# ahmetumutdurmus/zaremba

Measured on NVIDIA H100. Metric: tokens/sec (and valid perplexity) Large-LSTM 1500h at 1/2/4/8 H100 vs ref CPU, higher is better.
Workload: dtype f16 operands, f32 accumulate/state

## Files before the change

zaremba_b200/csrc/optim_tc.cu:

```cuda
#include "tc_kernels.h"

namespace zrb {

struct PackSpec {
    __half* row_img;
    int64_t ld;
    __half* fwd_img;
    int fU, fG, fKc, fKS;
    __half* bwd_img;
    int bUC, bG, bKc, bS;
    int write_g;
    int pdl;
};

__device__ __forceinline__ void pdl_prologue(const PackSpec& sp) {
    if (sp.pdl && threadIdx.x == 0) asm volatile("griddepcontrol.launch_dependents;" ::: "memory");
}
__device__ __forceinline__ void pdl_epilogue(const PackSpec& sp) {
    if (sp.pdl && blockIdx.x == 0 && threadIdx.x == 0) asm volatile("griddepcontrol.wait;" ::: "memory");
}

template <int VEC> struct VecT;
template <> struct VecT<4> { using type = float4; };
template <> struct VecT<2> { using type = float2; };
template <> struct VecT<1> { using type = float; };

template <int VEC>
__device__ __forceinline__ void load_vec(const float* p, float (&v)[VEC]) {
    typename VecT<VEC>::type t = __ldcs(reinterpret_cast<const typename VecT<VEC>::type*>(p));
    const float* f = reinterpret_cast<const float*>(&t);
#pragma unroll
    for (int i = 0; i < VEC; ++i) v[i] = f[i];
}
template <int VEC>
__device__ __forceinline__ void store_halves(__half* dst, const __half (&h)[VEC]) {
    if constexpr (VEC == 1) {
        dst[0] = h[0];
    } else {
#pragma unroll
        for (int x = 0; x < VEC; x += 2) reinterpret_cast<__half2*>(dst)[x >> 1] = __halves2half2(h[x], h[x + 1]);
    }
}

template <int VEC>
__device__ __forceinline__ void store_vec(float* p, const float (&v)[VEC]) {
    typename VecT<VEC>::type t;
    float* f = reinterpret_cast<float*>(&t);
#pragma unroll
    for (int i = 0; i < VEC; ++i) f[i] = v[i];
    __stcs(reinterpret_cast<typename VecT<VEC>::type*>(p), t);
}

struct SgdRule {
    float lr;
    const float* scalars;
    float coef;
    static constexpr bool kMayWriteG = true;
    __device__ __forceinline__ void init() { coef = scalars[1]; }
    template <int VEC>
    __device__ __forceinline__ void apply(int64_t, float (&pv)[VEC], float (&gv)[VEC]) const {
#pragma unroll
        for (int x = 0; x < VEC; ++x) { gv[x] *= coef; pv[x] = sgd_elem(pv[x], gv[x], lr); }
    }
};

template <bool RMS>
struct DynRule {
    const float* tg;
    const float* r;
    DynArgs a;
    float rbar;
    static constexpr bool kMayWriteG = false;
    __device__ __forceinline__ void init() { rbar = RMS ? *a.rbar : 0.f; }
    template <int VEC>
    __device__ __forceinline__ void apply(int64_t off, float (&pv)[VEC], float (&gv)[VEC]) const {
        float tv[VEC], rv[VEC];
        load_vec<VEC>(tg + off, tv);
        if constexpr (RMS) load_vec<VEC>(r + off, rv);
#pragma unroll
        for (int x = 0; x < VEC; ++x)
            pv[x] = dyneval_elem<RMS>(pv[x], gv[x], tv[x], RMS ? rv[x] : 0.f, a.lr, a.lam, a.eps, rbar);
    }
};

template <int VEC, class Rule>
__global__ void update_pack_kernel(float* __restrict__ p, float* __restrict__ g, int rows, int cols, Rule rule,
                                   PackSpec sp) {
    pdl_prologue(sp);
    rule.init();
    const int cv = cols / VEC;
    const int64_t total = (int64_t)rows * cv;
    for (int64_t i = (int64_t)blockIdx.x * blockDim.x + threadIdx.x; i < total; i += (int64_t)gridDim.x * blockDim.x) {
        const int r = (int)(i / cv), c = (int)(i % cv) * VEC;
        const int64_t off = (int64_t)r * cols + c;
        float gv[VEC], pv[VEC];
        load_vec<VEC>(g + off, gv);
        load_vec<VEC>(p + off, pv);
        rule.template apply<VEC>(off, pv, gv);
        if (Rule::kMayWriteG && sp.write_g) store_vec<VEC>(g + off, gv);
        store_vec<VEC>(p + off, pv);
        if (sp.row_img) {
            __half hh[VEC];
#pragma unroll
            for (int x = 0; x < VEC; ++x) hh[x] = __float2half_rn(pv[x]);
            store_halves<VEC>(sp.row_img + (int64_t)r * sp.ld + c, hh);
        }
    }
    pdl_epilogue(sp);
}

template <int VEC, class Rule>
__global__ void update_pack_whh_kernel(float* __restrict__ p, float* __restrict__ g, int H, Rule rule, PackSpec sp) {
    pdl_prologue(sp);
    rule.init();
    const int cv = H / VEC, jb_n = (H + 7) >> 3;
    const int64_t total = (int64_t)4 * jb_n * cv;
    for (int64_t i = (int64_t)blockIdx.x * blockDim.x + threadIdx.x; i < total; i += (int64_t)gridDim.x * blockDim.x) {
        const int c = (int)(i % cv) * VEC;
        const int jb = (int)((i / cv) % jb_n), q = (int)(i / ((int64_t)cv * jb_n));
        const int j0 = jb << 3;
        __half hv[8][VEC];
#pragma unroll
        for (int e = 0; e < 8; ++e) {
            const int j = j0 + e;
            if (j < H) {
                const int64_t off = ((int64_t)q * H + j) * H + c;
                float gv[VEC], pv[VEC];
                load_vec<VEC>(g + off, gv);
                load_vec<VEC>(p + off, pv);
                rule.template apply<VEC>(off, pv, gv);
#pragma unroll
                for (int x = 0; x < VEC; ++x) hv[e][x] = __float2half_rn(pv[x]);
                if (Rule::kMayWriteG && sp.write_g) store_vec<VEC>(g + off, gv);
                store_vec<VEC>(p + off, pv);
                if (sp.row_img) store_halves<VEC>(sp.row_img + ((int64_t)q * H + j) * sp.ld + c, hv[e]);
                if (sp.fwd_img) {
                    const int cluster = j / sp.fU, u = j % sp.fU, row = 4 * u + q;
                    const int kc = c >> 3, cta = cluster * sp.fKS + kc / sp.fKc, kcl = kc % sp.fKc;
                    store_halves<VEC>(sp.fwd_img + (((int64_t)cta * sp.fKc + kcl) * sp.fG + (row >> 3)) * 64 +
                                          (row & 7) * 8 + (c & 7), hv[e]);
                }
            } else {
#pragma unroll
                for (int x = 0; x < VEC; ++x) hv[e][x] = __float2half_rn(0.f);
            }
        }
        if (sp.bwd_img) {
#pragma unroll
            for (int x = 0; x < VEC; ++x) {
                const int cl = (c + x) / sp.bUC, u = (c + x) % sp.bUC;
                uint4 v;
                v.x = (uint32_t)__half_as_ushort(hv[0][x]) | ((uint32_t)__half_as_ushort(hv[1][x]) << 16);
                v.y = (uint32_t)__half_as_ushort(hv[2][x]) | ((uint32_t)__half_as_ushort(hv[3][x]) << 16);
                v.z = (uint32_t)__half_as_ushort(hv[4][x]) | ((uint32_t)__half_as_ushort(hv[5][x]) << 16);
                v.w = (uint32_t)__half_as_ushort(hv[6][x]) | ((uint32_t)__half_as_ushort(hv[7][x]) << 16);
                const int rank = q * sp.bS + jb / sp.bKc, kcl = jb % sp.bKc;
                *reinterpret_cast<uint4*>(sp.bwd_img + ((((int64_t)cl * 4 * sp.bS + rank) * sp.bKc + kcl) * sp.bG) * 64 +
                                          (u >> 3) * 64 + (u & 7) * 8) = v;
            }
        }
    }
    pdl_epilogue(sp);
}

template <int VEC, class Rule>
static int update_pack_launch(float* p, float* g, int rows, int cols, const Rule& rule, const PackSpec& sp, bool whh,
                              cudaStream_t s) {
    int64_t total = whh ? (int64_t)4 * ((cols + 7) / 8) * (cols / VEC) : (int64_t)rows * (cols / VEC);
    const int threads = whh ? 128 : 256;
    int blocks = (int)((total + threads - 1) / threads);
    if (blocks > 132 * 16) blocks = 132 * 16;
    if (sp.pdl) {
        cudaLaunchConfig_t cfg = {};
        cfg.gridDim = dim3(blocks); cfg.blockDim = dim3(threads); cfg.dynamicSmemBytes = 12 * 1024; cfg.stream = s;
        cudaLaunchAttribute at[1];
        at[0].id = cudaLaunchAttributeProgrammaticStreamSerialization;
        at[0].val.programmaticStreamSerializationAllowed = 1;
        cfg.attrs = at; cfg.numAttrs = 1;
        if (whh) ZRB_CUDA(cudaLaunchKernelEx(&cfg, update_pack_whh_kernel<VEC, Rule>, p, g, cols, rule, sp));
        else ZRB_CUDA(cudaLaunchKernelEx(&cfg, update_pack_kernel<VEC, Rule>, p, g, rows, cols, rule, sp));
        count_launch();
        return ZRB_OK;
    }
    if (whh) update_pack_whh_kernel<VEC, Rule><<<blocks, threads, 0, s>>>(p, g, cols, rule, sp);
    else update_pack_kernel<VEC, Rule><<<blocks, threads, 0, s>>>(p, g, rows, cols, rule, sp);
    ZRB_KERNEL_CHECK();
    return ZRB_OK;
}

template <class Rule>
static int update_pack_rule(float* p, float* g, int rows, int cols, const Rule& rule, uintptr_t align, __half* row_img,
                            int64_t ld, __half* fwd_img, const RecPlan* fp, __half* bwd_img, const RecPlan* bp,
                            bool write_g, cudaStream_t s, bool pdl) {
    PackSpec sp;
    sp.write_g = write_g ? 1 : 0;
    sp.pdl = pdl ? 1 : 0;
    sp.row_img = row_img; sp.ld = ld;
    sp.fwd_img = fwd_img; sp.fKS = fp ? fp->KS : 1; sp.fU = fp ? fp->KS * fp->U : 1; sp.fG = fp ? fp->G : 1;
    sp.fKc = fp ? fp->KcS : 1;
    sp.bwd_img = bwd_img; sp.bS = bp ? bp->KS : 1; sp.bUC = bp ? 4 * bp->KS * bp->U : 4; sp.bG = bp ? bp->G : 1;
    sp.bKc = bp ? bp->KcS : 1;
    const bool whh = (fwd_img || bwd_img) && rows == 4 * cols;
    const uintptr_t all = ((uintptr_t)p) | ((uintptr_t)g) | align;
    const bool al16 = (all & 15) == 0, al8 = (all & 7) == 0;
    if (cols % 4 == 0 && al16) return update_pack_launch<4>(p, g, rows, cols, rule, sp, whh, s);
    if (cols % 2 == 0 && al8) return update_pack_launch<2>(p, g, rows, cols, rule, sp, whh, s);
    return update_pack_launch<1>(p, g, rows, cols, rule, sp, whh, s);
}

int update_pack(float* p, float* g, int rows, int cols, float lr, const float* scalars, __half* row_img, int64_t ld,
                __half* fwd_img, const RecPlan* fp, __half* bwd_img, const RecPlan* bp, bool write_g, cudaStream_t s,
                bool pdl) {
    SgdRule rule;
    rule.lr = lr; rule.scalars = scalars; rule.coef = 0.f;
    return update_pack_rule(p, g, rows, cols, rule, 0, row_img, ld, fwd_img, fp, bwd_img, bp, write_g, s, pdl);
}

int update_pack_dyn(float* p, float* g, const float* tg, const float* r, int rows, int cols, const DynArgs& a,
                    __half* row_img, int64_t ld, __half* fwd_img, const RecPlan* fp, __half* bwd_img, const RecPlan* bp,
                    cudaStream_t s) {
    const uintptr_t align = ((uintptr_t)tg) | ((uintptr_t)r);
    if (a.rbar) {
        DynRule<true> rule{tg, r, a, 0.f};
        return update_pack_rule(p, g, rows, cols, rule, align, row_img, ld, fwd_img, fp, bwd_img, bp, false, s, false);
    }
    DynRule<false> rule{tg, nullptr, a, 0.f};
    return update_pack_rule(p, g, rows, cols, rule, align, row_img, ld, fwd_img, fp, bwd_img, bp, false, s, false);
}

}
```

Before: 364,800.

## Tile fused optimizer-update/pack kernels into 8-row blocks with warp-shuffled backward image stores

Replaces the grid-stride loops in the fused SGD/dynamic-eval update-and-pack kernels with a fixed 2D tiling: each thread handles an 8-row by VEC-column tile, batching all loads before the update math. In the W_hh kernel, the four gates q are mapped to adjacent lanes, and the backward-image 16-byte stores are reassembled via byte_perm and a lane-xor-4 shuffle so each thread writes contiguous units. It also adds launch bounds with per-rule min-blocks hints and uses vectorized half2 packing and stores. The aim is more memory-level parallelism and better-coalesced image writes in the per-step optimizer pass, at the cost of register pressure and more complex indexing.

```diff
diff --git a/zaremba_b200/csrc/optim_tc.cu b/zaremba_b200/csrc/optim_tc.cu
--- a/zaremba_b200/csrc/optim_tc.cu
+++ b/zaremba_b200/csrc/optim_tc.cu
@@ -32,14 +32,30 @@
 #pragma unroll
     for (int i = 0; i < VEC; ++i) v[i] = f[i];
 }
-template <int VEC>
-__device__ __forceinline__ void store_halves(__half* dst, const __half (&h)[VEC]) {
+__device__ __forceinline__ void st_v2(__half* dst, uint32_t a, uint32_t b) {
+    asm volatile("st.global.v2.b32 [%0], {%1, %2};" ::"l"(dst), "r"(a), "r"(b));
+}
+__device__ __forceinline__ void st_v4(__half* dst, const uint4& v) {
+    asm volatile("st.global.v4.b32 [%0], {%1, %2, %3, %4};" ::"l"(dst), "r"(v.x), "r"(v.y), "r"(v.z), "r"(v.w));
+}
+
+template <int VEC>
+__device__ __forceinline__ void pack_row(const float (&v)[VEC], uint32_t (&w)[(VEC + 1) / 2]) {
     if constexpr (VEC == 1) {
-        dst[0] = h[0];
+        w[0] = __half_as_ushort(__float2half_rn(v[0]));
     } else {
 #pragma unroll
-        for (int x = 0; x < VEC; x += 2) reinterpret_cast<__half2*>(dst)[x >> 1] = __halves2half2(h[x], h[x + 1]);
-    }
+        for (int k = 0; k < VEC / 2; ++k) {
+            const __half2 h = __floats2half2_rn(v[2 * k], v[2 * k + 1]);
+            w[k] = *reinterpret_cast<const uint32_t*>(&h);
+        }
+    }
+}
+template <int VEC>
+__device__ __forceinline__ void store_halves(__half* dst, const uint32_t (&w)[(VEC + 1) / 2]) {
+    if constexpr (VEC == 4) st_v2(dst, w[0], w[1]);
+    else if constexpr (VEC == 2) *reinterpret_cast<uint32_t*>(dst) = w[0];
+    else *reinterpret_cast<unsigned short*>(dst) = (unsigned short)w[0];
 }
 
 template <int VEC>
@@ -56,6 +72,7 @@
     const float* scalars;
     float coef;
     static constexpr bool kMayWriteG = true;
+    static constexpr int kWhhMinBlocks = 5;
     __device__ __forceinline__ void init() { coef = scalars[1]; }
     template <int VEC>
     __device__ __forceinline__ void apply(int64_t, float (&pv)[VEC], float (&gv)[VEC]) const {
@@ -71,6 +88,7 @@
     DynArgs a;
     float rbar;
     static constexpr bool kMayWriteG = false;
+    static constexpr int kWhhMinBlocks = 4;
     __device__ __forceinline__ void init() { rbar = RMS ? *a.rbar : 0.f; }
     template <int VEC>
     __device__ __forceinline__ void apply(int64_t off, float (&pv)[VEC], float (&gv)[VEC]) const {
@@ -83,80 +101,149 @@
     }
 };
 
+constexpr int kTileRows = 8;
+constexpr int kUpdThreads = 128;
+
 template <int VEC, class Rule>
-__global__ void update_pack_kernel(float* __restrict__ p, float* __restrict__ g, int rows, int cols, Rule rule,
-                                   PackSpec sp) {
+__device__ __forceinline__ void tile_update(const float* __restrict__ p, const float* __restrict__ g, int64_t off,
+                                            int stride, int n, const Rule& rule, float (&pv)[kTileRows][VEC],
+                                            float (&gv)[kTileRows][VEC]) {
+#pragma unroll
+    for (int e = 0; e < kTileRows; ++e) {
+        if (e < n) {
+            load_vec<VEC>(g + off + (int64_t)e * stride, gv[e]);
+            load_vec<VEC>(p + off + (int64_t)e * stride, pv[e]);
+        }
+    }
+#pragma unroll
+    for (int e = 0; e < kTileRows; ++e)
+        if (e < n) rule.template apply<VEC>(off + (int64_t)e * stride, pv[e], gv[e]);
+}
+
+template <int VEC>
+__device__ __forceinline__ void tile_store(float* __restrict__ p, float* __restrict__ g, int64_t off, int stride, int n,
+                                           bool write_g, const float (&pv)[kTileRows][VEC],
+                                           const float (&gv)[kTileRows][VEC]) {
+#pragma unroll
+    for (int e = 0; e < kTileRows; ++e) {
+        if (e < n) {
+            if (write_g) store_vec<VEC>(g + off + (int64_t)e * stride, gv[e]);
+            store_vec<VEC>(p + off + (int64_t)e * stride, pv[e]);
+        }
+    }
+}
+
+
+template <int VEC, class Rule>
+__global__ void __launch_bounds__(kUpdThreads) update_pack_kernel(float* __restrict__ p, float* __restrict__ g, int rows,
+                                                                  int cols, int col_tiles, Rule rule, PackSpec sp) {
     pdl_prologue(sp);
     rule.init();
-    const int cv = cols / VEC;
-    const int64_t total = (int64_t)rows * cv;
-    for (int64_t i = (int64_t)blockIdx.x * blockDim.x + threadIdx.x; i < total; i += (int64_t)gridDim.x * blockDim.x) {
-        const int r = (int)(i / cv), c = (int)(i % cv) * VEC;
-        const int64_t off = (int64_t)r * cols + c;
-        float gv[VEC], pv[VEC];
-        load_vec<VEC>(g + off, gv);
-        load_vec<VEC>(p + off, pv);
-        rule.template apply<VEC>(off, pv, gv);
-        if (Rule::kMayWriteG && sp.write_g) store_vec<VEC>(g + off, gv);
-        store_vec<VEC>(p + off, pv);
+    const unsigned rg = blockIdx.x / (unsigned)col_tiles, ct = blockIdx.x - rg * col_tiles;
+    const int c = (ct * blockDim.x + threadIdx.x) * VEC;
+    const int r0 = rg * kTileRows, n = min(kTileRows, rows - r0);
+    if (c < cols) {
+        const int64_t off = (int64_t)r0 * cols + c;
+        float pv[kTileRows][VEC], gv[kTileRows][VEC];
+        tile_update<VEC>(p, g, off, cols, n, rule, pv, gv);
+        tile_store<VEC>(p, g, off, cols, n, Rule::kMayWriteG && sp.write_g, pv, gv);
         if (sp.row_img) {
-            __half hh[VEC];
-#pragma unroll
-            for (int x = 0; x < VEC; ++x) hh[x] = __float2half_rn(pv[x]);
-            store_halves<VEC>(sp.row_img + (int64_t)r * sp.ld + c, hh);
+#pragma unroll
+            for (int e = 0; e < kTileRows; ++e) {
+                if (e < n) {
+                    uint32_t w[(VEC + 1) / 2];
+                    pack_row<VEC>(pv[e], w);
+                    store_halves<VEC>(sp.row_img + (int64_t)(r0 + e) * sp.ld + c, w);
+                }
+            }
         }
     }
     pdl_epilogue(sp);
 }
 
 template <int VEC, class Rule>
-__global__ void update_pack_whh_kernel(float* __restrict__ p, float* __restrict__ g, int H, Rule rule, PackSpec sp) {
+__global__ void __launch_bounds__(kUpdThreads, Rule::kWhhMinBlocks) update_pack_whh_kernel(float* __restrict__ p, float* __restrict__ g,
+                                                                      int H, int col_tiles, Rule rule, PackSpec sp) {
     pdl_prologue(sp);
     rule.init();
-    const int cv = H / VEC, jb_n = (H + 7) >> 3;
-    const int64_t total = (int64_t)4 * jb_n * cv;
-    for (int64_t i = (int64_t)blockIdx.x * blockDim.x + threadIdx.x; i < total; i += (int64_t)gridDim.x * blockDim.x) {
-        const int c = (int)(i % cv) * VEC;
-        const int jb = (int)((i / cv) % jb_n), q = (int)(i / ((int64_t)cv * jb_n));
-        const int j0 = jb << 3;
-        __half hv[8][VEC];
-#pragma unroll
-        for (int e = 0; e < 8; ++e) {
-            const int j = j0 + e;
-            if (j < H) {
-                const int64_t off = ((int64_t)q * H + j) * H + c;
-                float gv[VEC], pv[VEC];
-                load_vec<VEC>(g + off, gv);
-                load_vec<VEC>(p + off, pv);
-                rule.template apply<VEC>(off, pv, gv);
-#pragma unroll
-                for (int x = 0; x < VEC; ++x) hv[e][x] = __float2half_rn(pv[x]);
-                if (Rule::kMayWriteG && sp.write_g) store_vec<VEC>(g + off, gv);
-                store_vec<VEC>(p + off, pv);
-                if (sp.row_img) store_halves<VEC>(sp.row_img + ((int64_t)q * H + j) * sp.ld + c, hv[e]);
-                if (sp.fwd_img) {
-                    const int cluster = j / sp.fU, u = j % sp.fU, row = 4 * u + q;
-                    const int kc = c >> 3, cta = cluster * sp.fKS + kc / sp.fKc, kcl = kc % sp.fKc;
-                    store_halves<VEC>(sp.fwd_img + (((int64_t)cta * sp.fKc + kcl) * sp.fG + (row >> 3)) * 64 +
-                                          (row & 7) * 8 + (c & 7), hv[e]);
+    const int lane = threadIdx.x & 31, q = lane & 3;
+    const unsigned jb = blockIdx.x / (unsigned)col_tiles, ct = blockIdx.x - jb * col_tiles;
+    const int c = ((ct * (blockDim.x >> 5) + (threadIdx.x >> 5)) * 8 + (lane >> 2)) * VEC;
+    const int j0 = jb * kTileRows, n = min(kTileRows, H - j0);
+    uint32_t hw[kTileRows][(VEC + 1) / 2];
+    if (c < H) {
+        const int64_t off = ((int64_t)q * H + j0) * H + c;
+        float pv[kTileRows][VEC], gv[kTileRows][VEC];
+        tile_update<VEC>(p, g, off, H, n, rule, pv, gv);
+#pragma unroll
+        for (int e = 0; e < kTileRows; ++e) {
+            if (e < n) {
+                pack_row<VEC>(pv[e], hw[e]);
+            } else {
+#pragma unroll
+                for (int k = 0; k < (VEC + 1) / 2; ++k) hw[e][k] = 0;
+            }
+        }
+        tile_store<VEC>(p, g, off, H, n, Rule::kMayWriteG && sp.write_g, pv, gv);
+        if (sp.row_img) {
+#pragma unroll
+            for (int e = 0; e < kTileRows; ++e)
+                if (e < n) store_halves<VEC>(sp.row_img + (int64_t)(q * H + j0 + e) * sp.ld + c, hw[e]);
+        }
+        if (sp.fwd_img) {
+            const unsigned kc = (unsigned)c >> 3, kq = kc / (unsigned)sp.fKc, kcl = kc - kq * sp.fKc;
+            unsigned cluster = (unsigned)j0 / (unsigned)sp.fU, u = j0 - cluster * sp.fU;
+#pragma unroll
+            for (int e = 0; e < kTileRows; ++e) {
+                if (e < n) {
+                    const unsigned row = 4 * u + q, cta = cluster * sp.fKS + kq;
+                    store_halves<VEC>(sp.fwd_img + ((int64_t)(cta * sp.fKc + kcl) * sp.fG + (row >> 3)) * 64 +
+                                          (row & 7) * 8 + (c & 7), hw[e]);
                 }
-            } else {
-#pragma unroll
-                for (int x = 0; x < VEC; ++x) hv[e][x] = __float2half_rn(0.f);
-            }
-        }
-        if (sp.bwd_img) {
-#pragma unroll
-            for (int x = 0; x < VEC; ++x) {
-                const int cl = (c + x) / sp.bUC, u = (c + x) % sp.bUC;
-                uint4 v;
-                v.x = (uint32_t)__half_as_ushort(hv[0][x]) | ((uint32_t)__half_as_ushort(hv[1][x]) << 16);
-                v.y = (uint32_t)__half_as_ushort(hv[2][x]) | ((uint32_t)__half_as_ushort(hv[3][x]) << 16);
-                v.z = (uint32_t)__half_as_ushort(hv[4][x]) | ((uint32_t)__half_as_ushort(hv[5][x]) << 16);
-                v.w = (uint32_t)__half_as_ushort(hv[6][x]) | ((uint32_t)__half_as_ushort(hv[7][x]) << 16);
-                const int rank = q * sp.bS + jb / sp.bKc, kcl = jb % sp.bKc;
-                *reinterpret_cast<uint4*>(sp.bwd_img + ((((int64_t)cl * 4 * sp.bS + rank) * sp.bKc + kcl) * sp.bG) * 64 +
-                                          (u >> 3) * 64 + (u & 7) * 8) = v;
+                if (++u == (unsigned)sp.fU) { u = 0; ++cluster; }
+            }
+        }
+    } else {
+#pragma unroll
+        for (int e = 0; e < kTileRows; ++e)
+#pragma unroll
+            for (int k = 0; k < (VEC + 1) / 2; ++k) hw[e][k] = 0;
+    }
+    if (sp.bwd_img) {
+        uint4 v[VEC];
+#pragma unroll
+        for (int x = 0; x < VEC; ++x) {
+            uint32_t w[4];
+#pragma unroll
+            for (int m = 0; m < 4; ++m)
+                w[m] = VEC == 1 ? hw[2 * m][0] | (hw[2 * m + 1][0] << 16)
+                                : __byte_perm(hw[2 * m][x >> 1], hw[2 * m + 1][x >> 1], (x & 1) ? 0x7632 : 0x5410);
+            v[x] = make_uint4(w[0], w[1], w[2], w[3]);
+        }
+        const unsigned rank = q * sp.bS + jb / (unsigned)sp.bKc, kcl = jb - (jb / sp.bKc) * sp.bKc;
+        __half* base = sp.bwd_img + (int64_t)kcl * sp.bG * 64;
+        auto put = [&](int unit, const uint4& val) {
+            if (unit < H) {
+                const unsigned cl = (unsigned)unit / (unsigned)sp.bUC, u = unit - cl * sp.bUC;
+                st_v4(base + (int64_t)((cl * 4 * sp.bS + rank) * sp.bKc) * sp.bG * 64 + (u >> 3) * 64 + (u & 7) * 8, val);
+            }
+        };
+        if constexpr (VEC == 1) {
+            put(c, v[0]);
+        } else {
+            const bool lower = ((lane >> 2) & 1) == 0;
+            const int a = lower ? c : c - VEC;
+            uint4 recv[VEC / 2];
+#pragma unroll
+            for (int m = 0; m < VEC / 2; ++m) {
+                const uint4 s = lower ? v[2 * m + 1] : v[2 * m];
+                recv[m] = make_uint4(__shfl_xor_sync(0xffffffffu, s.x, 4), __shfl_xor_sync(0xffffffffu, s.y, 4),
+                                     __shfl_xor_sync(0xffffffffu, s.z, 4), __shfl_xor_sync(0xffffffffu, s.w, 4));
+            }
+#pragma unroll
+            for (int i = 0; i < VEC; ++i) {
+                if (lower) put(a + 2 * i, i < VEC / 2 ? v[2 * i] : recv[i - VEC / 2]);
+                else put(a + 2 * i + 1, i < VEC / 2 ? recv[i] : v[2 * (i - VEC / 2) + 1]);
             }
         }
     }
@@ -166,24 +253,29 @@
 template <int VEC, class Rule>
 static int update_pack_launch(float* p, float* g, int rows, int cols, const Rule& rule, const PackSpec& sp, bool whh,
                               cudaStream_t s) {
-    int64_t total = whh ? (int64_t)4 * ((cols + 7) / 8) * (cols / VEC) : (int64_t)rows * (cols / VEC);
-    const int threads = whh ? 128 : 256;
-    int blocks = (int)((total + threads - 1) / threads);
-    if (blocks > 132 * 16) blocks = 132 * 16;
+    const int cv = cols / VEC;
+    int threads = kUpdThreads, col_tiles;
+    if (whh) {
+        col_tiles = (cv + 8 * (threads / 32) - 1) / (8 * (threads / 32));
+    } else {
+        threads = min(kUpdThreads, (cv + 31) / 32 * 32);
+        col_tiles = (cv + threads - 1) / threads;
+    }
+    const dim3 grid((unsigned)(((rows / (whh ? 4 : 1)) + kTileRows - 1) / kTileRows * col_tiles));
     if (sp.pdl) {
         cudaLaunchConfig_t cfg = {};
-        cfg.gridDim = dim3(blocks); cfg.blockDim = dim3(threads); cfg.dynamicSmemBytes = 12 * 1024; cfg.stream = s;
+        cfg.gridDim = grid; cfg.blockDim = dim3(threads); cfg.dynamicSmemBytes = 12 * 1024; cfg.stream = s;
         cudaLaunchAttribute at[1];
         at[0].id = cudaLaunchAttributeProgrammaticStreamSerialization;
         at[0].val.programmaticStreamSerializationAllowed = 1;
         cfg.attrs = at; cfg.numAttrs = 1;
-        if (whh) ZRB_CUDA(cudaLaunchKernelEx(&cfg, update_pack_whh_kernel<VEC, Rule>, p, g, cols, rule, sp));
-        else ZRB_CUDA(cudaLaunchKernelEx(&cfg, update_pack_kernel<VEC, Rule>, p, g, rows, cols, rule, sp));
+        if (whh) ZRB_CUDA(cudaLaunchKernelEx(&cfg, update_pack_whh_kernel<VEC, Rule>, p, g, cols, col_tiles, rule, sp));
+        else ZRB_CUDA(cudaLaunchKernelEx(&cfg, update_pack_kernel<VEC, Rule>, p, g, rows, cols, col_tiles, rule, sp));
         count_launch();
         return ZRB_OK;
     }
-    if (whh) update_pack_whh_kernel<VEC, Rule><<<blocks, threads, 0, s>>>(p, g, cols, rule, sp);
-    else update_pack_kernel<VEC, Rule><<<blocks, threads, 0, s>>>(p, g, rows, cols, rule, sp);
+    if (whh) update_pack_whh_kernel<VEC, Rule><<<grid, threads, 0, s>>>(p, g, cols, col_tiles, rule, sp);
+    else update_pack_kernel<VEC, Rule><<<grid, threads, 0, s>>>(p, g, rows, cols, col_tiles, rule, sp);
     ZRB_KERNEL_CHECK();
     return ZRB_OK;
 }
```

After: 386,400, median of 6. 5.9% higher.
